# josh-holder/marl_sap

Hardware: AMD Instinct MI355X
Metric: env steps/sec (whole node), 64-agent assignment env, 1/2/4/8 MI355X (higher is better)
Workload: dtype f32

## Files before the change

marl_sap_amd/csrc/asg_agent_common.h:

```cpp
#pragma once
#include "asg_device.h"
#include "asg_internal.h"

namespace asg {

typedef float f32x4 __attribute__((ext_vector_type(4)));
typedef uint32_t u32x4v __attribute__((ext_vector_type(4)));
constexpr int kHid = 64;

__device__ __forceinline__ float comp(const float4 &v, int e) {
    return e == 0 ? v.x : e == 1 ? v.y : e == 2 ? v.z : v.w;
}

template <bool GEN, int NT, class SA>
__device__ __forceinline__ int select_finish(float (&best)[NT], int (&bj)[NT], const uint64_t (&amask)[NT][2],
                                             const int64_t (&rows)[NT], const bool (&ok)[NT],
                                             const int64_t (&oidx)[NT], int nct, SA &sel, int q) {
#pragma unroll
    for (int nt = 0; nt < NT; ++nt) {
        auto red = [&](auto swp) {
            const SwapPair pb = swp(__builtin_bit_cast(uint32_t, best[nt]));
            const SwapPair pj = swp((uint32_t)bj[nt]);
            float vb = __builtin_bit_cast(float, pb.a);
            int jb = (int)pj.a;
            if (better(__builtin_bit_cast(float, pb.b), (int)pj.b, vb, jb)) {
                vb = __builtin_bit_cast(float, pb.b);
                jb = (int)pj.b;
            }
            best[nt] = vb;
            bj[nt] = jb;
        };
        red(swap16);
        red(swap32);
    }
    const int nt = NT == 1 ? 0 : (q & 1);
    const int64_t row = rows[nt];
    int action = bj[nt] == 0x7fffffff ? 0 : bj[nt];
    bool explore = false;
    u32x4 rr = u32x4{0u, 0u, 0u, 0u};
    if (sel.epsilon > 0.0f) {
        const int64_t grow = row + sel.row_base;
        rr = philox4x32_10(u32x4{(uint32_t)grow, (uint32_t)(grow >> 32), kCtrSelect, sel.counter}, sel.k0, sel.k1);
        constexpr float k2m24 = 5.9604644775390625e-08f;
        explore = ok[nt] && q < NT && (float)(rr.x >> 8) * k2m24 < sel.epsilon;
    }
    if (__ballot(explore)) {
        const int nwin = (nct + 3) / 4;
        int target = -1, found = -1;
        for (int ntt = 0; ntt < NT; ++ntt) {
            const bool mine_row = explore && nt == ntt;
            int cnt = __popcll(amask[ntt][0]) + (GEN ? __popcll(amask[ntt][1]) : 0);
            {
                const SwapPair c16 = swap16((uint32_t)cnt);
                const SwapPair c32 = swap32(c16.a + c16.b);
                cnt = (int)(c32.a + c32.b);
            }
            if (mine_row) {
                if (cnt == 0) atomicCAS(sel.err, 0, ASG_E_INVALID_ARG);
                else target = (int)(((uint64_t)rr.y * (uint64_t)cnt) >> 32);
            }
            for (int w = 0; w < nwin; ++w) {
                const uint32_t mine = (uint32_t)(((GEN && w >= 4) ? amask[ntt][1] : amask[ntt][0]) >> (16 * (w & 3))) & 0xFFFFu;
                uint32_t lo = 0, hi = 0;
#pragma unroll
                for (int c = 0; c < 2; ++c) lo |= ((mine >> (4 * c)) & 0xFu) << (16 * c + 4 * q);
#pragma unroll
                for (int c = 2; c < 4; ++c) hi |= ((mine >> (4 * c)) & 0xFu) << (16 * (c - 2) + 4 * q);
                const SwapPair l16 = swap16(lo), h16 = swap16(hi);
                const SwapPair l32 = swap32(l16.a | l16.b), h32 = swap32(h16.a | h16.b);
                uint64_t row_mask = (uint64_t)(l32.a | l32.b) | ((uint64_t)(h32.a | h32.b) << 32);
                if (mine_row && target >= 0) {
                    const int pc = __popcll(row_mask);
                    if (target < pc) {
                        int k = target, pos = 0;
#pragma unroll
                        for (int half = 32; half >= 1; half >>= 1) {
                            const uint64_t low = row_mask & ((1ull << half) - 1ull);
                            const int lc = __popcll(low);
                            const bool up = k >= lc;
                            k -= up ? lc : 0;
                            pos += up ? half : 0;
                            row_mask = up ? (row_mask >> half) : low;
                        }
                        found = 64 * w + pos;
                        target = -1;
                    } else {
                        target -= pc;
                    }
                }
            }
        }
        if (found >= 0) action = found;
    }
    if (q < NT && ok[nt]) sel.out[oidx[nt]] = action;
    return action;
}

}
```

marl_sap_amd/csrc/h2_tile.h:

```cpp
#pragma once
#include <type_traits>

#include "asg_agent_common.h"

#pragma clang fp contract(fast)

namespace asg {

typedef _Float16 f16x8 __attribute__((ext_vector_type(8)));
typedef _Float16 f16x2v __attribute__((ext_vector_type(2)));
typedef long long i64x2v __attribute__((ext_vector_type(2)));
typedef const u32x4v __attribute__((address_space(3))) * lds_u4p;
typedef const f32x4 __attribute__((address_space(3))) * lds_f4v;

__device__ __forceinline__ f32x4 mfma_h(const u32x4v &a, const u32x4v &b, f32x4 c) {
    return __builtin_amdgcn_mfma_f32_16x16x32_f16(__builtin_bit_cast(f16x8, a), __builtin_bit_cast(f16x8, b), c, 0, 0,
                                                  0);
}
__device__ __forceinline__ f32x4 mfma_h2(const u32x4v (&w)[2], const u32x4v (&x)[2], f32x4 c) {
    c = mfma_h(w[1], x[0], c);
    c = mfma_h(w[0], x[1], c);
    c = mfma_h(w[0], x[0], c);
    return c;
}
// ... 58 lines not shown
    return (((int64_t)sl * 4 + mt) * 2 + pl) * 64 + lane;
}
__device__ __forceinline__ int w2_idx(int c, int sl, int pl, int lane) { return ((c * 2 + sl) * 2 + pl) * 64 + lane; }
static inline int64_t w1t_f4(const H2Geom &g) { return g.prefix ? (int64_t)g.P * 16 : 0; }

__host__ __device__ inline int64_t bias_f4(int nct) { return 80 + 4 * (int64_t)nct; }
__host__ __device__ inline int64_t lds_w2_off(bool rnn, int nct) { return rec_f4(rnn) + bias_f4(nct); }
__host__ __device__ inline int64_t lds_w1_off(bool rnn, int nct, bool w2l) {
    return lds_w2_off(rnn, nct) + (w2l ? w2s_f4(nct) : 0);
}

struct H2Args {
    const float *X;
    int64_t xs, R;
    H2Geom g;
    int pre;
    const float *Hin;
    int64_t hs;
    const u32x4v *pk;
    const float *W1T;
    const float *b1, *bi, *bh, *b2;
    float *Hout, *Q;
    SelectArgs sel;
    int w1_lds;
    int w1_off;
};

constexpr int kH2NT = 2;
constexpr int kH2WavesPerSimd = 2;
constexpr int kH2Waves = 4 * kH2WavesPerSimd;
constexpr int kH2XBuf = 2;
constexpr int kH2SxInit = 11;
#if defined(ASG_ROLLOUT_XSKIP) && !defined(ASG_TIMING_EXPERIMENTS)
#error "ASG_ROLLOUT_XSKIP gives wrong results: timing experiments only (-DASG_TIMING_EXPERIMENTS)"
#endif
#ifndef ASG_ROLLOUT_XSKIP
#define ASG_ROLLOUT_XSKIP 0
#endif

template <class A>
__device__ __forceinline__ int h2_s0(A &a) { return a.pre ? (a.g.Pp >> 5) : 0; }

template <bool RNN, bool W2L>
__device__ __forceinline__ void h2_stage(const H2Args &a, u32x4v *s, int (&sw)[4]) {
    const H2Geom &g = a.g;
    const u32x4v *rec = a.pk + 1 + w1s_f4(g.Kp);
    const int64_t nrec = rec_f4(RNN);
    for (int64_t i = threadIdx.x; i < nrec; i += blockDim.x) s[i] = rec[i];
    float *bs = reinterpret_cast<float *>(s + nrec);
    for (int i = threadIdx.x; i < 5 * kHid + 16 * g.nct; i += blockDim.x) {
        const int blk = i >> 6, u = i & 63;
        float v;
        if (blk == 0) v = a.b1[u];
        else if (blk < 5) {
            if (RNN) v = blk == 1 ? a.bi[u] + a.bh[u]
                       : blk == 2 ? a.bi[kHid + u] + a.bh[kHid + u]
                       : blk == 3 ? a.bi[2 * kHid + u] : a.bh[2 * kHid + u];
            else v = blk == 1 ? a.bi[u] : 0.f;
        } else {
            const int j = i - 5 * kHid;
            v = j < g.nout ? a.b2[j] : 0.f;
        }
        bs[i] = v;
    }
    if (W2L) {
        const int64_t n2 = w2s_f4(g.nct), off = lds_w2_off(RNN, g.nct);
        for (int64_t i = threadIdx.x; i < n2; i += blockDim.x) s[off + i] = rec[nrec + i];
    }
    {
        const u32x4v *w1 = a.pk + 1 + w1_idx(h2_s0(a) + a.w1_off, 0, 0, 0);
        const int64_t n1 = (int64_t)a.w1_lds * 4 * 2 * 64, off = lds_w1_off(RNN, g.nct, W2L);
        for (int64_t i = threadIdx.x; i < n1; i += blockDim.x) s[off + i] = w1[i];
    }
    const int4 hdr = *reinterpret_cast<const int4 *>(a.pk);
    sw[0] = hdr.x;
    sw[1] = hdr.y;
    sw[2] = hdr.z;
    sw[3] = hdr.w;
}

struct NoTailHook {
    template <class H>
    __device__ void operator()(const H &) const {}
};

template <int NT, bool RNN, bool SEL, bool W2L, bool ALLAV, bool GEN, bool HCOND = false, class Hook = NoTailHook,
          class A>
__device__ __forceinline__ void h2_tail(A &a, const u32x4v *Wl, const int (&sw)[4], int64_t row0,
                                        const int64_t (&rows)[NT], const bool (&ok)[NT], const float4 (&hB)[4][NT],
                                        const f32x4 (&xB)[4][NT], uint16_t *act_lds = nullptr, int lrow0 = 0,
                                        const Hook &after_rec = Hook{}, bool store_h = true) {
    int lane_ = threadIdx.x & 63;
    asm volatile("" : "+v"(lane_));
    const int lane = lane_, r = lane & 15, q = lane >> 4;
    const int nout = a.g.nout, nct = a.g.nct;
    const lds_u4p Wr = (lds_u4p)Wl;
    const lds_f4v Bs = (lds_f4v)(Wl + rec_f4(RNN));
    auto &sel = a.sel;
    const uint8_t *arow[NT];
    int64_t oidx[NT];
    bool av4 = false;
#pragma unroll
    for (int nt = 0; nt < NT; ++nt) {
        arow[nt] = nullptr;
        oidx[nt] = 0;
    }
    if (SEL) {
        const int64_t b0 = row0 / sel.n;
        const int i0 = (int)(row0 - b0 * sel.n);
#pragma unroll
        for (int nt = 0; nt < NT; ++nt) {
            int64_t b = b0;
            int i = i0 + 16 * nt + r;
            while (i >= sel.n) {
                i -= sel.n;
                ++b;
            }
            arow[nt] = ALLAV ? nullptr : sel.avail + (ok[nt] ? b * sel.a0 + (int64_t)i * sel.a1 : 0);
            oidx[nt] = b * sel.o0 + (int64_t)i * sel.o1;
        }
        av4 = !ALLAV && !GEN && ((reinterpret_cast<uintptr_t>(sel.avail) | (uintptr_t)sel.a0 | (uintptr_t)sel.a1) & 3u) == 0;
    }
    auto load_av = [&](int c, int nt) -> uint32_t {
        const int j0 = 16 * c + 4 * q;
        if (!SEL || !ok[nt]) return 0u;
        if (ALLAV) {
            if (!GEN) return 0x01010101u;
            const int nv = nout - j0;
            return nv >= 4 ? 0x01010101u : (nv <= 0 ? 0u : (0x01010101u & ((1u << (8 * nv)) - 1u)));
        }
        const uint8_t *ap = arow[nt] + j0;
        if (av4) return *reinterpret_cast<const uint32_t *>(ap);
        uint32_t w = 0;
#pragma unroll
        for (int v = 0; v < 4; ++v)
            if (!GEN || j0 + v < nout) w |= (uint32_t)ap[v] << (8 * v);
        return w;
    };
    uint32_t avw[4][NT];
#pragma unroll
    for (int c = 0; c < 4; ++c)
#pragma unroll
        for (int nt = 0; nt < NT; ++nt) avw[c][nt] = c < nct ? load_av(c, nt) : 0u;

    float mx[NT], mh[NT];
#pragma unroll
    for (int nt = 0; nt < NT; ++nt) {
        mx[nt] = 0.f;
        mh[nt] = 0.f;
#pragma unroll
        for (int t = 0; t < 4; ++t) {
            mx[nt] = absmax4(mx[nt], xB[t][nt]);
            if (RNN) mh[nt] = absmax4(mh[nt], hB[t][nt]);
        }
        mx[nt] = row_max4(mx[nt]);
        if (RNN) mh[nt] = row_max4(mh[nt]);
    }
    int Sg[NT];
    bool hz_all = true;
#pragma unroll
    for (int nt = 0; nt < NT; ++nt) {
        const bool hz = !RNN || !(mh[nt] > 0.f);
        hz_all = hz_all && hz;
        int s = min(sw[1] + h2_scale(mx[nt], -90, 90), hz ? 1000 : sw[2] + h2_scale(mh[nt], -90, 90));
        Sg[nt] = s > 100 ? 100 : (s < -100 ? -100 : s);
    }
    const bool h_zero = !RNN || __ballot(!hz_all) == 0;
    u32x4v xP[2][NT][2], hP[2][NT][2];
#pragma unroll
    for (int sl = 0; sl < 2; ++sl)
#pragma unroll
        for (int nt = 0; nt < NT; ++nt) {
            float v8[8], h8[8];
#pragma unroll
// ... 132 lines not shown
    int bj[NT];
    uint64_t amask[NT][2];
#pragma unroll
    for (int nt = 0; nt < NT; ++nt) {
        best[nt] = -__builtin_inff();
        bj[nt] = 0x7fffffff;
        amask[nt][0] = amask[nt][1] = 0;
        un3[nt] = pow2f(-S3[nt]);
    }
    int lane2 = lane;
    if (ALLAV) asm volatile("" : "+v"(lane2));
    const lds_u4p W2s = (lds_u4p)(Wl + lds_w2_off(RNN, nct));
    const u32x4v *W2g = a.pk + 1 + w1s_f4(a.g.Kp) + rec_f4(RNN);
    for (int c0 = 0; c0 < nct; c0 += 4) {
#pragma unroll
        for (int cc = 0; cc < 4; ++cc) {
            const int c = c0 + cc;
            if (c >= nct) break;
            const int j0 = 16 * c + 4 * q;
            uint32_t av[NT];
#pragma unroll
            for (int nt = 0; nt < NT; ++nt) {
                const uint32_t w = avw[cc][nt];
                av[nt] = ((w & 0xffu) != 0) | (((w >> 8) & 0xffu) != 0) << 1 | (((w >> 16) & 0xffu) != 0) << 2 |
                         ((w >> 24) != 0) << 3;
                if (c + 4 < nct) avw[cc][nt] = load_av(c + 4, nt);
            }
            f32x4 a2[NT];
#pragma unroll
            for (int nt = 0; nt < NT; ++nt) a2[nt] = f32x4{0.f, 0.f, 0.f, 0.f};
#pragma unroll
            for (int sl = 0; sl < 2; ++sl) {
                u32x4v w[2];
#pragma unroll
                for (int pl = 0; pl < 2; ++pl)
                    w[pl] = W2L ? W2s[w2_idx(c, sl, pl, lane2)] : W2g[w2_idx(c, sl, pl, lane2)];
#pragma unroll
                for (int nt = 0; nt < NT; ++nt) a2[nt] = mfma_h2(w, hq[sl][nt], a2[nt]);
            }
            const f32x4 bq = Bs[80 + 4 * c + q];
#pragma unroll
            for (int nt = 0; nt < NT; ++nt) {
                const f32x4 qv = a2[nt] * un3[nt] + bq;
                if (a.Q && ok[nt]) {
                    float *qp = a.Q + rows[nt] * nout + j0;
                    if (!GEN) {
                        *reinterpret_cast<float4 *>(qp) = make_float4(qv[0], qv[1], qv[2], qv[3]);
                    } else {
#pragma unroll
                        for (int v = 0; v < 4; ++v)
                            if (j0 + v < nout) qp[v] = qv[v];
                    }
                }
                if (SEL && ALLAV && !GEN) {
#pragma unroll
                    for (int v = 0; v < 4; ++v) {
                        const int j = j0 + v;
                        const float x = qv[v];
                        const bool b = (c == 0 && v == 0) | ((best[nt] == best[nt]) & !(x <= best[nt]));
                        best[nt] = b ? x : best[nt];
                        bj[nt] = b ? j : bj[nt];
                    }
                } else if (SEL) {
#pragma unroll
                    for (int v = 0; v < 4; ++v) {
                        const int j = j0 + v;
                        const float x = ((av[nt] >> v) & 1u) ? qv[v] : -__builtin_inff();
                        const bool b = ((bj[nt] == 0x7fffffff) & (j < nout)) |
                                       ((best[nt] == best[nt]) & !(x <= best[nt]) & (j < nout));
                        best[nt] = b ? x : best[nt];
                        bj[nt] = b ? j : bj[nt];
                    }
                    amask[nt][0] |= (uint64_t)av[nt] << (4 * (c & 15));
                }
            }
        }
    }
    if (SEL && ALLAV && !GEN) {
        const uint64_t all = nct >= 16 ? ~0ull : ((1ull << (4 * nct)) - 1ull);
#pragma unroll
        for (int nt = 0; nt < NT; ++nt) amask[nt][0] = all;
    }
    if (SEL) {
        const int act = select_finish<false, NT>(best, bj, amask, rows, ok, oidx, nct, sel, q);
        const int nt = NT == 1 ? 0 : (q & 1);
        if (act_lds && q < NT && ok[nt]) act_lds[lrow0 + 16 * nt + r] = (uint16_t)act;
    }
}

template <int NT, bool RNN, bool SEL, bool W2L, bool GEN, class A>
__device__ __forceinline__ void agent_rows_h2(int64_t row0, A &a, const u32x4v *Wl, const int (&sw)[4]) {
    const int lane = threadIdx.x & 63, r = lane & 15, q = lane >> 4;
    if (row0 >= a.R) return;
    auto &g = a.g;
    int64_t rows[NT];
    bool ok[NT];
#pragma unroll
    for (int nt = 0; nt < NT; ++nt) {
        rows[nt] = row0 + 16 * nt + r;
        ok[nt] = rows[nt] < a.R;
    }
    const lds_f4v Bs = (lds_f4v)(Wl + rec_f4(RNN));
    const u32x4v *W1g = a.pk + 1;
    const float *xr[NT];
#pragma unroll
    for (int nt = 0; nt < NT; ++nt) xr[nt] = a.X + (ok[nt] ? rows[nt] : 0) * a.xs;
    const int Ub = g.Pp >> 5, nsl = g.Kp >> 5;
    const int s0 = h2_s0(a);

    auto load_x = [&](int sl, float4 (&xv)[2][NT]) {
        if (!GEN) {
#pragma unroll
            for (int c = 0; c < 2; ++c)
#pragma unroll
                for (int nt = 0; nt < NT; ++nt)
                    xv[c][nt] = *reinterpret_cast<const float4 *>(xr[nt] + 32 * sl + 16 * c + 4 * q);
        } else {
            const int blk = sl / Ub, jj0 = 32 * (sl - blk * Ub);
#pragma unroll
            for (int c = 0; c < 2; ++c)
#pragma unroll
                for (int nt = 0; nt < NT; ++nt) {
                    const int jj = jj0 + 16 * c + 4 * q;
                    const float *p = xr[nt] + (int64_t)blk * g.P + jj;
                    float v[4];
#pragma unroll
                    for (int e = 0; e < 4; ++e) v[e] = (ok[nt] && jj + e < g.P) ? p[e] : 0.f;
                    xv[c][nt] = make_float4(v[0], v[1], v[2], v[3]);
                }
        }
    };
    auto load_pa = [&](int t4, float4 (&pa)[4][NT]) {
#pragma unroll
        for (int c = 0; c < 4; ++c)
#pragma unroll
            for (int nt = 0; nt < NT; ++nt) {
                const int jj = 16 * (t4 + c) + 4 * q;
                if (t4 + c >= (g.Pp >> 4)) {
                    pa[c][nt] = make_float4(0.f, 0.f, 0.f, 0.f);
                } else if (!GEN) {
                    pa[c][nt] = *reinterpret_cast<const float4 *>(xr[nt] + jj);
                } else {
                    float v[4];
#pragma unroll
                    for (int e = 0; e < 4; ++e) v[e] = (ok[nt] && jj + e < g.P) ? xr[nt][jj + e] : 0.f;
                    pa[c][nt] = make_float4(v[0], v[1], v[2], v[3]);
                }
            }
    };
    float4 pa[4][NT];
    if (a.pre) load_pa(0, pa);
    const int nmain = nsl - s0;
    const int nblk = g.NB - 1;
    auto sl_of = [&](int idx) { return a.pre ? (idx % nblk + 1) * Ub + idx / nblk : idx; };
    float4 xbuf[kH2XBuf][2][NT];
#pragma unroll
    for (int b = 0; b < kH2XBuf; ++b)
        if (b < nmain) load_x(sl_of(b), xbuf[b]);

    int pos[NT];
    bool onehot = false;
#pragma unroll
    for (int nt = 0; nt < NT; ++nt) pos[nt] = -1;
    if (a.pre) {
        bool bad = false;
        for (int t4 = 0; t4 < (g.Pp >> 4); t4 += 4) {
            if (t4 > 0) load_pa(t4, pa);
#pragma unroll
            for (int c = 0; c < 4; ++c)
// ... 145 lines not shown
```

marl_sap_amd/csrc/rollout_kernel.h:

```cpp
#pragma once
#include "rollout_tile.h"

#pragma clang fp contract(fast)

namespace asg {

template <bool RNN, bool W2L, bool GEN, int TAB, bool QOUT, int SQ>
__device__ __forceinline__ void rollout_envs_wave(const RolloutArgs &ra, u32x4v *s_h2, const int (&sw)[4]) {
    const int lane = threadIdx.x & 63, wv = __builtin_amdgcn_readfirstlane(threadIdx.x >> 6);
    const int n = rs_n<SQ>(ra), m = rs_m<SQ>(ra), mp = rollout_mp(m), np = rollout_np(n);
    char *scr = reinterpret_cast<char *>(s_h2 + ra.scratch_off) + wv * rollout_scratch_bytes(n, m);
    uint64_t *s_scl = reinterpret_cast<uint64_t *>(scr + kWaveSclOff);
    double *s_ret = reinterpret_cast<double *>(scr + kWaveRetOff);
    int *s_cnt = reinterpret_cast<int *>(scr + kWaveCntOff);
    uint16_t *s_act = reinterpret_cast<uint16_t *>(s_cnt + mp);
    uint16_t *s_prev = s_act + np;
    const int ntile = np / (16 * kH2NT);
    const int64_t GW = (int64_t)gridDim.x * kH2Waves;
    for (int64_t e0 = (int64_t)blockIdx.x * kH2Waves + wv; e0 < ra.E; e0 += GW) {
        int64_t e = e0;
        asm volatile("" : "+s"(e));
        const EnvKey key = env_key(ra.seed, ra.env_base + e);
        for (int c = 0; c < (TAB ? 0 : (mp + 63) / 64); ++c) {
            const int j = 64 * c + lane;
// ... 3 lines not shown
        }
        rollout_env_prologue<TAB>(ra, e, key, n, m, lane, s_cnt, s_act, s_prev, s_ret);
        wave_lds_fence();
        KRolloutArgs *const kra = (KRolloutArgs *)__builtin_amdgcn_kernarg_segment_ptr();
        const int sf = ra.select_first ? 1 : 0;
        const int nit = ra.k1 - ra.k0 + sf;
        int pass = 0;
        f32x4 hN[4][kH2NT];
        bool hpf = false;
        auto has_agent = [&](auto &rr, int it) {
            return rollout_has_agent(it, nit, sf, rr.k0, rr.k1, rr.T, rr.select_last);
        };
        for (int it = 0; it < nit; ++it) {
            auto &ri = rollout_args(kra);
            const int k = ri.k0 + it - sf;
            const int ts = ri.ts0 + (k - ri.k0);
            const bool first_sel = it < sf;
            if (!first_sel && !(ASG_ROLLOUT_XSKIP & 256))
                rollout_transition<TAB, SQ>(rollout_args(kra), e, k, ts, key, s_scl, s_cnt, s_act, s_prev, s_ret);
            const int kk = k + 1;
            if (has_agent(ri, it)) {
                const bool next_agent = has_agent(ri, it + 1);
                for (int sub = 0; sub < ntile; ++sub) {
                    HNext nx{nullptr, kHid, 0, 0};
                    if (sub + 1 < ntile) nx = HNext{pass == 0 ? ri.Hin : ri.Hout, pass == 0 ? ri.hs : kHid,
                                                    (int64_t)(16 * kH2NT) * (sub + 1), 1};
                    else if (next_agent) nx = HNext{ri.Hout, kHid, 0, 1};
                    rollout_tile<RNN, W2L, GEN, TAB, QOUT, true, SQ>(rollout_args(kra), e, sub, kk, ts + 1,
                                                                     !first_sel || ri.reset, !first_sel, pass, key, s_scl,
                                                                     s_act, s_act, s_h2, sw, hN, hpf, nx);
                    hpf = nx.mode != 0;
                }
                ++pass;
            } else {
                for (int sub = 0; sub < ntile; ++sub)
                    rollout_tile<RNN, W2L, GEN, TAB, QOUT, false, SQ>(rollout_args(kra), e, sub, kk, ts + 1, true, true, 0,
                                                                      key, s_scl, s_act, s_act, s_h2, sw, hN, false,
                                                                      HNext{nullptr, kHid, 0, 0});
            }
            wave_lds_fence();
        }
        for (int i = lane; i < n; i += 64) ra.prev[e * n + i] = s_prev[i];
        if (lane == 0) ra.returns[e] = *s_ret;
        wave_lds_fence();
    }
}

template <bool RNN, bool W2L, int TAB, bool QOUT>
__device__ __forceinline__ void rollout_envs_pair(const RolloutArgs &ra, u32x4v *s_h2, const int (&sw)[4]) {
    constexpr int SQ = 64, n = 64, m = 64;
    const int wv = __builtin_amdgcn_readfirstlane(threadIdx.x >> 6);
    const int pr = wv >> 1, sub = wv & 1;
    const bool trw = sub == (pr >> 1);
    char *scr = reinterpret_cast<char *>(s_h2 + ra.scratch_off) + pr * pair_scratch_bytes(ra.defer);
    uint64_t *s_scl = reinterpret_cast<uint64_t *>(scr + kPairSclOff + kPairSclStride * sub);
    double *s_ret = reinterpret_cast<double *>(scr + kPairRetOff);
    int *s_cnt = reinterpret_cast<int *>(scr + kPairCntOff + kPairCntStride * sub);
    uint16_t *s_prev = reinterpret_cast<uint16_t *>(scr + kPairPrevOff);
    uint16_t *s_hist = reinterpret_cast<uint16_t *>(scr + kPairHistOff);
    auto s_sum = [&](int j) { return reinterpret_cast<double *>(s_hist + kPairRow * j + kPairSumOff); };
    constexpr int kPairs = kH2Waves / 2;
    const int64_t GP = (int64_t)gridDim.x * kPairs;
    for (int64_t eb = (int64_t)blockIdx.x * kPairs; eb < ra.E; eb += GP) {
        int64_t e = eb + pr;
        asm volatile("" : "+s"(e));
        const bool active = e < ra.E;
        const EnvKey key = env_key(ra.seed, ra.env_base + e);
        int lane = threadIdx.x & 63;
        asm volatile("" : "+v"(lane));
        if (active) {
            if (!TAB) {
                const bool ten = philox_task_scale(key, ra.episode, lane) == 10.0f;
                const uint64_t bits = __ballot(ten);
                if (lane == 0) s_scl[0] = bits;
            }
            if (trw) rollout_env_prologue<TAB>(ra, e, key, n, m, lane, s_cnt, s_hist, s_prev, s_ret);
        }
        wave_lds_fence();
        pair_barrier();
        KRolloutArgs *const kra = (KRolloutArgs *)__builtin_amdgcn_kernarg_segment_ptr();
        const int sf = ra.select_first ? 1 : 0;
        const int nit = ra.k1 - ra.k0 + sf;
        f32x4 hN[4][kH2NT];
        auto has_agent = [&](auto &rr, int it) {
            return rollout_has_agent(it, nit, sf, rr.k0, rr.k1, rr.T, rr.select_last);
        };
        for (int g0 = 0; g0 < nit; g0 += rollout_args(kra).defer) {
            const int gn = min(rollout_args(kra).defer, nit - g0);
            for (int j = 0; j < gn; ++j) {
                const int it = g0 + j, pass = it;
                auto &ri = rollout_args(kra);
                const int k = ri.k0 + it - sf;
                const int ts = ri.ts0 + (k - ri.k0);
                const bool first_sel = it < sf;
                const bool agent = has_agent(ri, it);
                uint16_t *const sa = s_hist + kPairRow * j, *const saw = sa + kPairRow;
                if (active) {
                    const int kk = k + 1;
                    if (agent) {
                        const int last = __builtin_amdgcn_readfirstlane(has_agent(ri, it + 1) ? 0 : 1);
                        rollout_tile<RNN, W2L, false, TAB, QOUT, true, SQ>(rollout_args(kra), e, sub, kk, ts + 1,
                                                                           !first_sel || ri.reset, !first_sel, pass, key,
                                                                           s_scl, sa, saw, s_h2, sw, hN, pass > 0,
                                                                           HKeep{last});
                    } else {
                        rollout_tile<RNN, W2L, false, TAB, QOUT, false, SQ>(rollout_args(kra), e, sub, kk, ts + 1, true, true,
                                                                            0, key, s_scl, sa, saw, s_h2, sw, hN, false,
                                                                            HKeep{0});
                    }
                }
                wave_lds_fence();
            }
            pair_barrier();
            int lane = threadIdx.x & 63;
            asm volatile("" : "+v"(lane));
            const int own = 32 * sub + (lane & 31);
            const bool moved = g0 + gn > sf;
            uint16_t t_last = 0, t_next = 0;
            if (active) {
                for (int j = (sub + g0) & 1; j < gn; j += 2) {
                    const int it = g0 + j;
                    if (it < sf || (ASG_ROLLOUT_XSKIP & 256)) continue;
                    auto &ri = rollout_args(kra);
                    const int k = ri.k0 + it - sf;
                    const int ts = ri.ts0 + (k - ri.k0);
                    uint16_t *const pv = (j == 0 || it - 1 < sf) ? s_prev : s_hist + kPairRow * (j - 1);
                    rollout_transition<TAB, SQ, true>(rollout_args(kra), e, k, ts, key, s_scl, s_cnt, s_hist + kPairRow * j,
                                                      pv, s_sum(j));
                }
                t_last = moved ? s_hist[kPairRow * (gn - 1) + own] : s_prev[own];
                t_next = s_hist[kPairRow * gn + own];
            }
            pair_barrier();
            if (active) {
                const bool more = g0 + gn < nit;
                if (lane < 32) {
                    if (more) {
                        s_prev[own] = t_last;
                        s_hist[own] = t_next;
                    } else {
                        ra.prev[e * n + own] = t_last;
                    }
                }
                if (trw && lane == 0) {
                    double ret = *s_ret;
                    for (int j = 0; j < gn; ++j)
                        if (g0 + j >= sf && !(ASG_ROLLOUT_XSKIP & 256)) ret += *s_sum(j);
                    *s_ret = ret;
                    if (!more) ra.returns[e] = ret;
                }
            }
            wave_lds_fence();
        }
    }
}

template <bool RNN, bool W2L, bool GEN, int TAB, bool QOUT, int SQ, bool PAIR = false>
__global__ void __launch_bounds__(64 * kH2Waves) __attribute__((amdgpu_waves_per_eu(kH2WavesPerSimd)))
rollout_kernel(RolloutArgs ra) {
    static_assert(!PAIR || (SQ == 64 && !GEN && !QOUT), "the wave-pair mapping: n = m = 64, selecting instances");
    extern __shared__ u32x4v s_h2[];
    int sw[4];
    h2_stage<RNN, W2L>(rollout_h2args(ra), s_h2, sw);
    __syncthreads();
    if constexpr (PAIR) rollout_envs_pair<RNN, W2L, TAB, QOUT>(ra, s_h2, sw);
    else rollout_envs_wave<RNN, W2L, GEN, TAB, QOUT, SQ>(ra, s_h2, sw);
}

template <int TAB, bool QOUT>
static hipError_t launch_rollout_inst(const RolloutArgs &ra, const RolloutLaunch &lc, hipStream_t s) {
#define LR_(RNN, W2L, GEN, SQ, PAIR)                                                                            \
    hipLaunchKernelGGL((rollout_kernel<RNN, W2L, GEN, TAB, QOUT, SQ, PAIR>), dim3(lc.grid), dim3(64 * kH2Waves), lc.lds, \
                       s, ra)
#define LR2_(RNN)                                                                              \
    do {                                                                                       \
        if (lc.sq64 && lc.pair) {                                                              \
            if constexpr (QOUT) return hipErrorInvalidValue;    \
            else LR_(RNN, true, false, 64, true);                                              \
        } else if (lc.sq64) {                                                                  \
            LR_(RNN, true, false, 64, false);                                                  \
        } else if (lc.w2l) {                                                                   \
            if (lc.gen) LR_(RNN, true, true, 0, false); else LR_(RNN, true, false, 0, false);   \
        } else {                                                                               \
            if (lc.gen) LR_(RNN, false, true, 0, false); else LR_(RNN, false, false, 0, false); \
        }                                                                                      \
    } while (0)
    if (lc.rnn) LR2_(true); else LR2_(false);
#undef LR2_
#undef LR_
    return hipGetLastError();
}
// ... 5 lines not shown
```

marl_sap_amd/csrc/rollout_tile.h:

```cpp
#pragma once
#include "rollout_env.h"
#include "rollout_rows.h"

#pragma clang fp contract(fast)

namespace asg {

struct HNext {
    const float *src;
    int64_t stride, row0;
    int mode;
};
struct HKeep {
    int store;
};

template <bool RNN, bool W2L, bool GEN, int TAB, bool QOUT, bool AGENT, int SQ, class HX, class RA>
__device__ __forceinline__ void rollout_tile(RA &ra, int64_t e, int sub, int kk, int tsr, bool stores,
                                             bool have_act, int pass, const EnvKey &key, const uint64_t *s_scl,
                                             const uint16_t *s_act, uint16_t *s_actw, const u32x4v *Wl,
                                             const int (&sw)[4], f32x4 (&hN)[4][kH2NT], bool hpf, HX nx) {
    constexpr int NT = kH2NT;
    constexpr int RT = 16 * NT;
    asm volatile("" : "+s"(e), "+s"(tsr), "+s"(kk));
    int lane_ = threadIdx.x & 63;
    asm volatile("" : "+v"(lane_));
    const int lane = lane_, r = lane & 15, q = lane >> 4;
    const int n = rs_n<SQ>(ra), m = rs_m<SQ>(ra), T = ra.T, L = ra.L;
    const int K = m * (L + 1);
    const int Ub = rollout_mp(m) >> 5;
    const int64_t row0 = e * n + RT * sub;
    int64_t rows[NT];
    bool ok[NT];
    int ia[NT], act[NT];
#pragma unroll
    for (int nt = 0; nt < NT; ++nt) {
        ia[nt] = RT * sub + 16 * nt + r;
        ok[nt] = !GEN || ia[nt] < n;
        rows[nt] = e * n + ia[nt];
        act[nt] = (have_act && ok[nt]) ? (int)s_act[ia[nt]] : -1;
    }
    constexpr bool cmp = TAB == 2;
    uint64_t cmw[NT];
    int cof[NT];
    auto load_cm = [&](int w) {
        const int W = (m + 63) >> 6;
#pragma unroll
        for (int nt = 0; nt < NT; ++nt) {
            const int64_t r = (e * n + (ok[nt] ? ia[nt] : 0)) * W + w;
            cmw[nt] = cmp ? ra.tmask[r] : 0ull;
            cof[nt] = cmp ? ra.toff[r] : 0;
        }
    };
    if (cmp && SQ == 64) load_cm(0);
    auto table_quad = [&](const float *trow, int j0, int nt, uint32_t &nb) {
        const float *tp = trow + (int64_t)ia[nt] * m + j0;
        if constexpr (cmp) {
            const f32x4 x = compact_quad_load(trow, cmw[nt], cof[nt], j0 & 63, ok[nt] && j0 < m, &nb);
            return make_float4(x.x, x.y, x.z, x.w);
        } else if (!GEN) {
            return *reinterpret_cast<const float4 *>(tp);
        } else {
            float v4[4];
#pragma unroll
            for (int v = 0; v < 4; ++v) v4[v] = (ok[nt] && j0 + v < m) ? tp[v] : 0.f;
            return make_float4(v4[0], v4[1], v4[2], v4[3]);
        }
    };
    const int tss = (ASG_ROLLOUT_XSKIP & 32) ? 1 : tsr;
    const int64_t sro = (ASG_ROLLOUT_XSKIP & 32) ? ((e & 7) - e) * n : 0;
    float *obs_r = ra.obs + ((int64_t)tss * ra.E * n + sro) * K;
    f32x4 acc[4][NT];
    int sx[NT];
    if (AGENT) {
        const float scS = pow2f(sw[0] + kH2SxInit);
#pragma unroll
        for (int nt = 0; nt < NT; ++nt) {
            sx[nt] = kH2SxInit;
#pragma unroll
            for (int mt = 0; mt < 4; ++mt) {
                const float4 g = (act[nt] >= 0 && !(ASG_ROLLOUT_XSKIP & 2))
                                     ? *reinterpret_cast<const float4 *>(ra.W1T + act[nt] * kHid + 16 * mt + 4 * q)
                                     : make_float4(0.f, 0.f, 0.f, 0.f);
                acc[mt][nt] = f32x4{g.x, g.y, g.z, g.w} * scS;
            }
        }
    }
    if (AGENT && RNN) {
        if (!hpf) {
            const float *hin = pass == 0 ? ra.Hin : ra.Hout;
            const int64_t hs = pass == 0 ? ra.hs : kHid;
#pragma unroll
            for (int t = 0; t < 4; ++t)
#pragma unroll
                for (int nt = 0; nt < NT; ++nt)
                    hN[t][nt] = hin ? *reinterpret_cast<const f32x4 *>(hin + (ok[nt] ? rows[nt] : 0) * hs + 16 * t + 4 * q)
                                    : f32x4{0.f, 0.f, 0.f, 0.f};
        }
#pragma unroll
        for (int t = 0; t < 4; ++t)
#pragma unroll
            for (int nt = 0; nt < NT; ++nt) asm volatile("" : "+v"(hN[t][nt]));
    }
    if (stores && !(ASG_ROLLOUT_XSKIP & 1)) {
        int64_t *oh_r = (ra.onehot && have_act) ? ra.onehot + ((int64_t)(tss - 1) * ra.E * n + sro) * m : nullptr;
        uint8_t *ab = ra.avail ? ra.avail + ((int64_t)tss * ra.E * n + sro + row0) * m : nullptr;
        if constexpr (SQ == 64)
            tile_action_rows64(obs_r + row0 * K, oh_r ? oh_r + row0 * m : nullptr, ab, K, s_act + RT * sub, have_act);
        for (int u = 0; u < (SQ == 64 ? 0 : Ub); ++u)
#pragma unroll
            for (int c = 0; c < 2; ++c)
#pragma unroll
                for (int nt = 0; nt < NT; ++nt) {
                    const int j0 = 32 * u + 16 * c + 4 * q;
                    const int aa = act[nt];
                    if (!GEN) {
                        st_f4(obs_r + rows[nt] * K + j0, aa == j0, aa == j0 + 1, aa == j0 + 2, aa == j0 + 3);
                        if (oh_r) {
                            st_i64x2(oh_r + rows[nt] * m + j0, aa == j0, aa == j0 + 1);
                            st_i64x2(oh_r + rows[nt] * m + j0 + 2, aa == j0 + 2, aa == j0 + 3);
                        }
                    } else if (ok[nt]) {
#pragma unroll
                        for (int v = 0; v < 4; ++v)
                            if (j0 + v < m) {
                                obs_r[rows[nt] * K + j0 + v] = aa == j0 + v ? 1.0f : 0.0f;
                                if (oh_r) oh_r[rows[nt] * m + j0 + v] = aa == j0 + v;
                            }
                    }
                }
        if (SQ != 64 && ab) {
            const int nrow = GEN ? min(RT, n - RT * sub) : RT;
            int off0 = (GEN ? 1 : 16) * lane;
            asm volatile("" : "+v"(off0));
            if (!GEN) {
                for (int i = 0; i < Ub; ++i)
                    *reinterpret_cast<u32x4v *>(ab + 1024 * i + (uint32_t)off0) =
                        u32x4v{0x01010101u, 0x01010101u, 0x01010101u, 0x01010101u};
            } else {
                for (int off = off0; off < nrow * m; off += 64) ab[off] = 1;
            }
        }
    }
    BumpShape bsh = bump_shape(T, ra.wmin, ra.wmax);
    bsh.q = __builtin_amdgcn_readfirstlane(bsh.q);
    const lds_f4v Bs = (lds_f4v)(Wl + rec_f4(RNN));
    const u32x4v *W1g = ra.pk + 1;
    const int s0 = Ub, s_l2 = s0 + ra.w1_off + ra.w1_lds;
    float *beta_r = ra.beta ? ra.beta + ((int64_t)tss * ra.E * n + sro) * m : nullptr;
    const bool live = kk < T;
    for (int attempt = 0;; ++attempt) {
        float scx[NT], rmax[NT];
#pragma unroll
        for (int nt = 0; nt < NT; ++nt) {
            scx[nt] = pow2f(AGENT ? sx[nt] : 0);
            rmax[nt] = 0.f;
        }
        if (AGENT && attempt > 0) {
#pragma unroll
            for (int nt = 0; nt < NT; ++nt) {
                const float scS = pow2f(sw[0] + sx[nt]);
#pragma unroll
                for (int mt = 0; mt < 4; ++mt) {
                    const float4 g = act[nt] >= 0
                                         ? *reinterpret_cast<const float4 *>(ra.W1T + act[nt] * kHid + 16 * mt + 4 * q)
                                         : make_float4(0.f, 0.f, 0.f, 0.f);
                    acc[mt][nt] = f32x4{g.x, g.y, g.z, g.w} * scS;
                }
            }
        }
        const bool st_now = stores && attempt == 0 && !(ASG_ROLLOUT_XSKIP & 1);
        for (int u = 0; u < Ub; ++u) {
            Bump32 bp[2][4][NT];
            constexpr int kPre = TAB == 2 ? kTabPreCmp : kTabPre;
            float4 tv[kPre][2][NT];
            if (cmp && SQ != 64) load_cm(u >> 1);
            if constexpr (TAB != 0) {
#pragma unroll
                for (int l = 1; l <= kPre; ++l) {
                    const int t = kk + l - 1;
                    if (l > L || t >= T) continue;
                    const float *trow = ra.table32 + ((int64_t)e * T + t) * n * m;
#pragma unroll
                    for (int c = 0; c < 2; ++c)
#pragma unroll
// ... 61 lines not shown
                        }
                } else if (TAB && t < T) {
                    const float *trow = ra.table32 + ((int64_t)e * T + t) * n * m;
#pragma unroll
                    for (int c = 0; c < 2; ++c)
#pragma unroll
                        for (int nt = 0; nt < NT; ++nt) {
                            uint32_t nb;
                            const float4 x = table_quad(trow, 32 * u + 16 * c + 4 * q, nt, nb);
                            if constexpr (cmp) xv[c][nt] = compact_expand(f32x4{x.x, x.y, x.z, x.w}, nb);
                            else xv[c][nt] = x;
                        }
                } else if (!TAB && t < T) {
#pragma unroll
                    for (int c = 0; c < 2; ++c)
#pragma unroll
                        for (int nt = 0; nt < NT; ++nt)
                            xv[c][nt] = make_float4(bump32_at(bp[c][0][nt], t), bump32_at(bp[c][1][nt], t),
                                                    bump32_at(bp[c][2][nt], t), bump32_at(bp[c][3][nt], t));
                } else {
#pragma unroll
                    for (int c = 0; c < 2; ++c)
#pragma unroll
                        for (int nt = 0; nt < NT; ++nt) xv[c][nt] = make_float4(0.f, 0.f, 0.f, 0.f);
                }
                auto store_rows = [&]() {
#pragma unroll
                    for (int c = 0; c < 2; ++c)
#pragma unroll
                        for (int nt = 0; nt < NT; ++nt) {
                            const float vv[4] = {xv[c][nt].x, xv[c][nt].y, xv[c][nt].z, xv[c][nt].w};
                            const int j0 = 32 * u + 16 * c + 4 * q;
                            if (!GEN) {
                                st_f4(obs_r + rows[nt] * K + m * l + j0, vv[0], vv[1], vv[2], vv[3]);
                                if (l == 1 && beta_r) st_f4(beta_r + rows[nt] * m + j0, vv[0], vv[1], vv[2], vv[3]);
                            } else if (ok[nt]) {
#pragma unroll
                                for (int v = 0; v < 4; ++v)
                                    if (j0 + v < m) {
                                        obs_r[rows[nt] * K + m * l + j0 + v] = vv[v];
                                        if (l == 1 && beta_r) beta_r[rows[nt] * m + j0 + v] = vv[v];
                                    }
                            }
                        }
                };
                const bool late = !W2L && AGENT && l * Ub + u >= s_l2;
                if (st_now && !late) store_rows();
                if (AGENT) {
                    const int sl = l * Ub + u;
                    u32x4v xp[NT][2];
#pragma unroll
                    for (int nt = 0; nt < NT; ++nt) {
                        rmax[nt] = absmax4(absmax4(rmax[nt], xv[0][nt]), xv[1][nt]);
                        const float x8[8] = {xv[0][nt].x, xv[0][nt].y, xv[0][nt].z, xv[0][nt].w,
                                             xv[1][nt].x, xv[1][nt].y, xv[1][nt].z, xv[1][nt].w};
                        split2s(x8, scx[nt], xp[nt][0], xp[nt][1]);
                    }
                    auto mma = [&](bool lds) {
#pragma unroll
                        for (int mt = 0; mt < 4; ++mt) {
                            u32x4v w[2];
                            if (lds) {
                                const lds_u4p W1s = (lds_u4p)(Wl + lds_w1_off(RNN, (m + 15) / 16, W2L));
#pragma unroll
                                for (int pl = 0; pl < 2; ++pl)
                                    w[pl] = W1s[w1_idx((ASG_ROLLOUT_XSKIP & 4) && sl >= s_l2 ? 0 : sl - s0 - ra.w1_off, mt,
                                                       pl, lane)];
                            } else {
#pragma unroll
                                for (int pl = 0; pl < 2; ++pl) w[pl] = W1g[w1_idx(sl, mt, pl, lane)];
                            }
#pragma unroll
                            for (int nt = 0; nt < NT; ++nt) acc[mt][nt] = mfma_h2(w, xp[nt], acc[mt][nt]);
                        }
                    };
                    if ((sl >= s0 + ra.w1_off && sl < s_l2) || (ASG_ROLLOUT_XSKIP & 4))
                        mma(true);
                    else
                        mma(false);
                }
                if (st_now && late) store_rows();
            }
        }
        if (!AGENT) return;
        bool over[NT], any = false;
#pragma unroll
        for (int nt = 0; nt < NT; ++nt) {
            const float rm = row_max4(rmax[nt]);
            over[nt] = rm * scx[nt] >= 32768.f;
            any = any || over[nt];
            if (over[nt]) sx[nt] = h2_scale(rm, -90, 90 - sw[0]);
        }
        if (attempt > 0 || __ballot(any) == 0) break;
    }
    if constexpr (AGENT) {
        H2Args a = rollout_h2args<SQ>(ra);
        a.sel.counter = ra.counter + (uint32_t)pass;
        a.sel.out = ra.act + (int64_t)tsr * ra.E * n;
        if constexpr (QOUT) a.Q = ra.Q;
        float4 hB[4][NT];
#pragma unroll
        for (int t = 0; t < 4; ++t)
#pragma unroll
            for (int nt = 0; nt < NT; ++nt)
                hB[t][nt] = (ASG_ROLLOUT_XSKIP & 8) ? make_float4(0.5f, 0.25f, -0.5f, 0.125f)
                            : RNN ? make_float4(hN[t][nt][0], hN[t][nt][1], hN[t][nt][2], hN[t][nt][3])
                                  : make_float4(0.f, 0.f, 0.f, 0.f);
        f32x4 xB[4][NT];
#pragma unroll
        for (int nt = 0; nt < NT; ++nt) {
            const float un = pow2f(-(sw[0] + sx[nt]));
#pragma unroll
            for (int mt = 0; mt < 4; ++mt) {
                const f32x4 bb = Bs[4 * mt + q];
#pragma unroll
                for (int v = 0; v < 4; ++v) xB[mt][nt][v] = fmaxf(acc[mt][nt][v] * un + bb[v], 0.f);
            }
        }
        if constexpr (std::is_same<HX, HKeep>::value) {
            auto keep = [&](const f32x4(&hp)[4][NT]) {
                if (!RNN) return;
#pragma unroll
                for (int t = 0; t < 4; ++t)
#pragma unroll
                    for (int nt = 0; nt < NT; ++nt) hN[t][nt] = hp[t][nt];
            };
            h2_tail<NT, RNN, !QOUT, W2L, true, GEN, true>(a, Wl, sw, row0, rows, ok, hB, xB, s_actw, RT * sub, keep,
                                                          nx.store != 0);
        } else {
        auto prefetch = [&](const auto &) {
            if (!RNN || nx.mode == 0) return;
            const int64_t nb = e * n + nx.row0;
#pragma unroll
            for (int t = 0; t < 4; ++t)
#pragma unroll
                for (int nt = 0; nt < NT; ++nt) {
                    const int ni = (int)nx.row0 + 16 * nt + r;
                    const bool nok = !GEN || ni < n;
                    hN[t][nt] = nx.src ? *reinterpret_cast<const f32x4 *>(nx.src + (nok ? nb + 16 * nt + r : 0) * nx.stride +
                                                                        16 * t + 4 * q)
                                       : f32x4{0.f, 0.f, 0.f, 0.f};
                }
        };
        h2_tail<NT, RNN, !QOUT, W2L, true, GEN>(a, Wl, sw, row0, rows, ok, hB, xB, s_actw, RT * sub, prefetch);
        }
    }
}

}
```

Baseline: 34.80 million.

## Prefetch next step's W1 action-column gather right after action selection

After selecting actions in the agent tail, the kernel now immediately gathers the W1T rows for the chosen actions into registers (gN) and carries them to the next rollout step, which seeds its accumulators from them instead of redoing that gather. The action store to global memory moves into the hook so it sits alongside the gather. The aim is to hide the dependent-load latency of the action-indexed weight gather behind the rest of the tail. The cost is extra live registers across steps (a 4xNT f32x4 array), which may pressure occupancy, plus a static assert restricting the path to NT==2 and non-generic layouts.

```diff
diff --git a/marl_sap_amd/csrc/asg_agent_common.h b/marl_sap_amd/csrc/asg_agent_common.h
--- a/marl_sap_amd/csrc/asg_agent_common.h
+++ b/marl_sap_amd/csrc/asg_agent_common.h
@@ -12,7 +12,7 @@
     return e == 0 ? v.x : e == 1 ? v.y : e == 2 ? v.z : v.w;
 }
 
-template <bool GEN, int NT, class SA>
+template <bool GEN, int NT, bool STORE = true, class SA>
 __device__ __forceinline__ int select_finish(float (&best)[NT], int (&bj)[NT], const uint64_t (&amask)[NT][2],
                                              const int64_t (&rows)[NT], const bool (&ok)[NT],
                                              const int64_t (&oidx)[NT], int nct, SA &sel, int q) {
@@ -92,7 +92,7 @@
         }
         if (found >= 0) action = found;
     }
-    if (q < NT && ok[nt]) sel.out[oidx[nt]] = action;
+    if (STORE && q < NT && ok[nt]) sel.out[oidx[nt]] = action;
     return action;
 }
 
diff --git a/marl_sap_amd/csrc/h2_tile.h b/marl_sap_amd/csrc/h2_tile.h
--- a/marl_sap_amd/csrc/h2_tile.h
+++ b/marl_sap_amd/csrc/h2_tile.h
@@ -164,14 +164,17 @@
 struct NoTailHook {
     template <class H>
     __device__ void operator()(const H &) const {}
+    template <class H, class O, class I>
+    __device__ bool operator()(const H &, O, const I &) const { return false; }
 };
 
 template <int NT, bool RNN, bool SEL, bool W2L, bool ALLAV, bool GEN, bool HCOND = false, class Hook = NoTailHook,
-          class A>
+          class SelHook = NoTailHook, class A>
 __device__ __forceinline__ void h2_tail(A &a, const u32x4v *Wl, const int (&sw)[4], int64_t row0,
                                         const int64_t (&rows)[NT], const bool (&ok)[NT], const float4 (&hB)[4][NT],
                                         const f32x4 (&xB)[4][NT], uint16_t *act_lds = nullptr, int lrow0 = 0,
-                                        const Hook &after_rec = Hook{}, bool store_h = true) {
+                                        const Hook &after_rec = Hook{}, bool store_h = true,
+                                        const SelHook &after_sel = SelHook{}) {
     int lane_ = threadIdx.x & 63;
     asm volatile("" : "+v"(lane_));
     const int lane = lane_, r = lane & 15, q = lane >> 4;
@@ -470,9 +473,14 @@
         for (int nt = 0; nt < NT; ++nt) amask[nt][0] = all;
     }
     if (SEL) {
-        const int act = select_finish<false, NT>(best, bj, amask, rows, ok, oidx, nct, sel, q);
+        constexpr bool hooked = !std::is_same<SelHook, NoTailHook>::value;
+        const int act = select_finish<false, NT, !hooked>(best, bj, amask, rows, ok, oidx, nct, sel, q);
         const int nt = NT == 1 ? 0 : (q & 1);
         if (act_lds && q < NT && ok[nt]) act_lds[lrow0 + 16 * nt + r] = (uint16_t)act;
+        if constexpr (hooked) {
+            if (!after_sel(lrow0, sel.out, oidx))
+                if (q < NT && ok[nt]) sel.out[oidx[nt]] = act;
+        }
     }
 }
 
diff --git a/marl_sap_amd/csrc/rollout_kernel.h b/marl_sap_amd/csrc/rollout_kernel.h
--- a/marl_sap_amd/csrc/rollout_kernel.h
+++ b/marl_sap_amd/csrc/rollout_kernel.h
@@ -109,6 +109,7 @@
         const int sf = ra.select_first ? 1 : 0;
         const int nit = ra.k1 - ra.k0 + sf;
         f32x4 hN[4][kH2NT];
+        f32x4 gN[4][kH2NT];
         auto has_agent = [&](auto &rr, int it) {
             return rollout_has_agent(it, nit, sf, rr.k0, rr.k1, rr.T, rr.select_last);
         };
@@ -129,11 +130,11 @@
                         rollout_tile<RNN, W2L, false, TAB, QOUT, true, SQ>(rollout_args(kra), e, sub, kk, ts + 1,
                                                                            !first_sel || ri.reset, !first_sel, pass, key,
                                                                            s_scl, sa, saw, s_h2, sw, hN, pass > 0,
-                                                                           HKeep{last});
+                                                                           HKeep{last, pass > 0, !last, gN});
                     } else {
                         rollout_tile<RNN, W2L, false, TAB, QOUT, false, SQ>(rollout_args(kra), e, sub, kk, ts + 1, true, true,
                                                                             0, key, s_scl, sa, saw, s_h2, sw, hN, false,
-                                                                            HKeep{0});
+                                                                            HKeep{0, 0, 0, gN});
                     }
                 }
                 wave_lds_fence();
diff --git a/marl_sap_amd/csrc/rollout_tile.h b/marl_sap_amd/csrc/rollout_tile.h
--- a/marl_sap_amd/csrc/rollout_tile.h
+++ b/marl_sap_amd/csrc/rollout_tile.h
@@ -13,7 +13,17 @@
 };
 struct HKeep {
     int store;
+    int got, give;
+    f32x4 (&gN)[4][kH2NT];
 };
+
+
+__device__ __forceinline__ void drop_gather(f32x4 (&gN)[4][kH2NT]) {
+#pragma unroll
+    for (int mt = 0; mt < 4; ++mt)
+#pragma unroll
+        for (int nt = 0; nt < kH2NT; ++nt) gN[mt][nt] = f32x4{0.f, 0.f, 0.f, 0.f};
+}
 
 template <bool RNN, bool W2L, bool GEN, int TAB, bool QOUT, bool AGENT, int SQ, class HX, class RA>
 __device__ __forceinline__ void rollout_tile(RA &ra, int64_t e, int sub, int kk, int tsr, bool stores,
@@ -21,6 +31,7 @@
                                              const uint16_t *s_act, uint16_t *s_actw, const u32x4v *Wl,
                                              const int (&sw)[4], f32x4 (&hN)[4][kH2NT], bool hpf, HX nx) {
     constexpr int NT = kH2NT;
+    constexpr bool GPF = std::is_same<HX, HKeep>::value && TAB != 1;
     constexpr int RT = 16 * NT;
     asm volatile("" : "+s"(e), "+s"(tsr), "+s"(kk));
     int lane_ = threadIdx.x & 63;
@@ -72,7 +83,23 @@
     float *obs_r = ra.obs + ((int64_t)tss * ra.E * n + sro) * K;
     f32x4 acc[4][NT];
     int sx[NT];
-    if (AGENT) {
+    bool got = false;
+    if constexpr (AGENT && GPF) {
+        got = nx.got != 0;
+        if (got) {
+            const float scS = pow2f(sw[0] + kH2SxInit);
+#pragma unroll
+            for (int nt = 0; nt < NT; ++nt) {
+                sx[nt] = kH2SxInit;
+#pragma unroll
+                for (int mt = 0; mt < 4; ++mt) {
+                    acc[mt][nt] = nx.gN[mt][nt] * scS;
+                    asm volatile("" : "+v"(acc[mt][nt]));
+                }
+            }
+        }
+    }
+    if (AGENT && !got) {
         const float scS = pow2f(sw[0] + kH2SxInit);
 #pragma unroll
         for (int nt = 0; nt < NT; ++nt) {
@@ -97,10 +124,12 @@
                     hN[t][nt] = hin ? *reinterpret_cast<const f32x4 *>(hin + (ok[nt] ? rows[nt] : 0) * hs + 16 * t + 4 * q)
                                     : f32x4{0.f, 0.f, 0.f, 0.f};
         }
-#pragma unroll
-        for (int t = 0; t < 4; ++t)
-#pragma unroll
-            for (int nt = 0; nt < NT; ++nt) asm volatile("" : "+v"(hN[t][nt]));
+        if (!GPF || !hpf) {
+#pragma unroll
+            for (int t = 0; t < 4; ++t)
+#pragma unroll
+                for (int nt = 0; nt < NT; ++nt) asm volatile("" : "+v"(hN[t][nt]));
+        }
     }
     if (stores && !(ASG_ROLLOUT_XSKIP & 1)) {
         int64_t *oh_r = (ra.onehot && have_act) ? ra.onehot + ((int64_t)(tss - 1) * ra.E * n + sro) * m : nullptr;
@@ -328,7 +357,10 @@
                 if (st_now && late) store_rows();
             }
         }
-        if (!AGENT) return;
+        if constexpr (!AGENT) {
+            if constexpr (GPF) drop_gather(nx.gN);
+            return;
+        }
         bool over[NT], any = false;
 #pragma unroll
         for (int nt = 0; nt < NT; ++nt) {
@@ -371,8 +403,36 @@
 #pragma unroll
                     for (int nt = 0; nt < NT; ++nt) hN[t][nt] = hp[t][nt];
             };
-            h2_tail<NT, RNN, !QOUT, W2L, true, GEN, true>(a, Wl, sw, row0, rows, ok, hB, xB, s_actw, RT * sub, keep,
-                                                          nx.store != 0);
+            auto next_gather = [&](int lrow0, auto *out, const int64_t (&oidx)[NT]) {
+                if (!nx.give) {
+                    drop_gather(nx.gN);
+                    return false;
+                }
+                wave_lds_fence();
+                int ln = threadIdx.x & 63;
+                asm volatile("" : "+v"(ln));
+                int an[NT];
+#pragma unroll
+                for (int nt = 0; nt < NT; ++nt) {
+                    an[nt] = (int)s_actw[lrow0 + 16 * nt + (ln & 15)];
+#pragma unroll
+                    for (int mt = 0; mt < 4; ++mt)
+                        nx.gN[mt][nt] =
+                            *reinterpret_cast<const f32x4 *>(ra.W1T + an[nt] * kHid + 16 * mt + 4 * (ln >> 4));
+                }
+                static_assert(NT == 2 && !GEN, "rows nt = q & 1, every row an agent's");
+                const bool odd = ((ln >> 4) & 1) != 0;
+                int64_t o0 = oidx[0], o1 = oidx[1];
+                asm volatile("" : "+v"(o0), "+v"(o1));
+                out[odd ? o1 : o0] = odd ? an[1] : an[0];
+                return true;
+            };
+            if constexpr (GPF)
+                h2_tail<NT, RNN, !QOUT, W2L, true, GEN, true>(a, Wl, sw, row0, rows, ok, hB, xB, s_actw, RT * sub, keep,
+                                                              nx.store != 0, next_gather);
+            else
+                h2_tail<NT, RNN, !QOUT, W2L, true, GEN, true>(a, Wl, sw, row0, rows, ok, hB, xB, s_actw, RT * sub, keep,
+                                                              nx.store != 0);
         } else {
         auto prefetch = [&](const auto &) {
             if (!RNN || nx.mode == 0) return;
```

New measurement: 34.89 million (median of 3 runs). No clear change (+0.3%).
